# Vinmwaura/Quantized-Autoregression-Image-Generator

Hardware: NVIDIA B200
Metric: patches/sec BMU+update (SOM training step P=4 D=64 K=16384, 1 048 576 patches per step over all GPUs) (higher is better)
Workload: dtype f32 (BMU: fp16 hi/lo split x3 products on tcgen05, fp32 accumulate; update, filters and Adam fp32; filters 3xTF32)

## Files before the change

### quantized-autoregression-image-generator_b200/csrc/som_bmu_tc_l16.cu

```cuda
#include "som_common.cuh"
#include "som_tc_ptx.cuh"
#include "som_tc_split.cuh"

namespace som {
SOM_TRACE_TU(trace_set_l16)
namespace tcl16 {
using namespace tc;

constexpr int NA_MAX = 4;
constexpr int NB_MAX = 8;
constexpr int BUILD_WARP0 = 2, BUILD_WARPS = 4;
constexpr int EPI_WARP0 = 6, EPI_WARPS = 8;
constexpr int NUM_THREADS = (EPI_WARP0 + EPI_WARPS) * 32;
constexpr int A_SLOT_BYTES = 2 * A_BLK_BYTES;
constexpr int TAIL_A_BYTES = TM * 32;
constexpr int TAIL_B_BYTES = TN * 32;
constexpr int DMAX = 256;
constexpr int RING_BYTES = 192 * 1024;
constexpr int TILES_BYTES = RING_BYTES + 2 * TAIL_A_BYTES + 2 * TAIL_B_BYTES;

struct Params {
    int DB;
    int nks_last;
    int NT;
    int n_mtiles;
    int NA, NB;
    int K_pad;
    int64_t rows;
    int64_t unit_offset;
    int64_t* out_idx;
    float* out_rd;
    const void* x;
    Geom g;
    const float* scale;
    float* stage;
    const uint32_t* wflags;
};

struct __align__(8) Barriers {
    uint64_t b_full[NB_MAX], b_empty[NB_MAX];
    uint64_t t_full[2], t_empty[2];
    uint64_t a_full[NA_MAX], a_empty[NA_MAX];
    uint64_t acc_full[2], acc_empty[2];
    uint64_t exp_full[2];
    uint32_t tmem_base, pad;
};
struct Aux {
    Barriers bars;
    int foff[DMAX];
    float mrg_val[2][TM];
    int mrg_idx[2][TM];
    int row_exp[2][TM];
    alignas(8) uint8_t lo_nz[NA_MAX][8];
};
constexpr uint32_t SMEM_BYTES = 1024 + TILES_BYTES + sizeof(Aux);
constexpr int WFLAG_WORDS_MAX = 1024;
constexpr uint32_t SMEM_BYTES_W16 = SMEM_BYTES + WFLAG_WORDS_MAX * 4;
static_assert(SMEM_BYTES_W16 <= 227 * 1024, "FP16-split kernel: shared memory over the 227 KB limit");

__device__ long long g_prof16[8];

template <int CG, bool MERGED, typename T, bool W16 = false>
__global__ void __launch_bounds__(NUM_THREADS, 1)
bmu_tc_l16_kernel(const __grid_constant__ CUtensorMap map_b, const __grid_constant__ CUtensorMap map_t, const Params P) {
    constexpr bool IN16 = sizeof(T) == 2;
    pdl_launch_dependents();
    extern __shared__ uint8_t smem_raw[];
    uint8_t* tiles = aligned_tiles(smem_raw);
    constexpr int B_STAGE = B_BLK_BYTES / CG;
    constexpr int T_STAGE = TAIL_B_BYTES / CG;
    constexpr int M_STAGE = 2 * B_STAGE + T_STAGE;
    const int NA = P.NA, NB = P.NB, DB = P.DB;
    uint8_t* a_ring = tiles;
    uint8_t* a_tail = MERGED ? tiles + 2 * A_SLOT_BYTES : tiles + RING_BYTES;
    uint8_t* b_ring = MERGED ? a_tail + 2 * TAIL_A_BYTES : a_ring + (size_t)NA * A_SLOT_BYTES;
    uint8_t* t_ring = a_tail + 2 * TAIL_A_BYTES;
    Aux& aux = *reinterpret_cast<Aux*>(tiles + TILES_BYTES);
    Barriers& bars = aux.bars;
    const uint32_t rank = (CG == 2) ? cluster_ctarank() : 0u;
    const int job0 = (CG == 2) ? (int)cluster_id_x() : (int)blockIdx.x;
    const int job_stride = (CG == 2) ? (int)cluster_count_x() : (int)gridDim.x;
    const int n_jobs = (P.n_mtiles + CG - 1) / CG;

    const int warp = threadIdx.x >> 5;
    const int lane = threadIdx.x & 31;
    const int D = P.g.D;

    if (threadIdx.x == 0) {
        for (int s = 0; s < NB_MAX; ++s) { mbar_init(&bars.b_full[s], 1); mbar_init(&bars.b_empty[s], 1); }
        for (int s = 0; s < 2; ++s) { mbar_init(&bars.t_full[s], 1); mbar_init(&bars.t_empty[s], 1); }
        for (int s = 0; s < NA_MAX; ++s) { mbar_init(&bars.a_full[s], BUILD_WARPS * CG); mbar_init(&bars.a_empty[s], 1); }
        for (int a = 0; a < 2; ++a) {
            mbar_init(&bars.acc_full[a], 1);
            mbar_init(&bars.acc_empty[a], EPI_WARPS * CG);
            mbar_init(&bars.exp_full[a], BUILD_WARPS);
        }
        if (IN16)
            for (int s = 0; s < NA_MAX; ++s) *reinterpret_cast<uint64_t*>(aux.lo_nz[s]) = 0ull;
        asm volatile("fence.mbarrier_init.release.cluster;" ::: "memory");
    }
    for (int d = threadIdx.x; d < D; d += NUM_THREADS) aux.foff[d] = feat_off(P.g, d);
    if (CG == 2) {
        __syncthreads();
        cluster_sync_all();
    }
    if (warp == 1) tmem_alloc<CG>(&bars.tmem_base, 512);
    tc_fence_before();
    __syncthreads();
    if (CG == 2) cluster_sync_all();
    tc_fence_after();
    const uint32_t tmem_base = bars.tmem_base;
    pdl_wait();
    trace_stamp(s_trace_buf, 7);
    uint32_t* wbits = reinterpret_cast<uint32_t*>(tiles + TILES_BYTES + sizeof(Aux));
    if (W16) {
        for (int w = threadIdx.x; w < (P.NT * DB + 31) >> 5; w += NUM_THREADS) wbits[w] = P.wflags[w];
        __syncthreads();
    }
    auto b_lo = [&](int n, int fb) -> bool {
        if (!W16) return true;
        const int b = n * DB + fb;
        return (wbits[b >> 5] >> (b & 31)) & 1u;
    };

    if (warp == 0) {
        if (lane == 0) {
            int bs = 0, ts = 0;
            uint32_t b_ph = 0, t_ph = 0;
            const int row_off = (int)rank * (TN / CG);
            for (int q = job0; q < n_jobs; q += job_stride) {
                for (int n = 0; n < P.NT; ++n) {
                    if (MERGED) {
                        for (int fb = 0; fb < DB; ++fb) {
                            const bool blo = b_lo(n, fb);
                            mbar_wait(&bars.b_empty[bs], b_ph ^ 1);
                            if (rank == 0)
                                mbar_expect_tx(&bars.b_full[bs], (blo ? 2 : 1) * B_BLK_BYTES + (fb == 0 ? TAIL_B_BYTES : 0));
                            uint8_t* dst = b_ring + (size_t)bs * M_STAGE;
#pragma unroll
                            for (int part = 0; part < 2; ++part) {
                                if (part == 1 && !blo) break;
                                if (CG == 1) tma_load_2d(&map_b, &bars.b_full[bs], dst + part * B_STAGE, (part * DB + fb) * KBLK, n * TN);
                                else tma_load_2d_pair(&map_b, &bars.b_full[bs], dst + part * B_STAGE, (part * DB + fb) * KBLK, n * TN + row_off);
                            }
                            if (fb == 0) {
                                if (CG == 1) tma_load_2d(&map_t, &bars.b_full[bs], dst + 2 * B_STAGE, 0, n * TN);
                                else tma_load_2d_pair(&map_t, &bars.b_full[bs], dst + 2 * B_STAGE, 0, n * TN + row_off);
                            }
                            if (++bs == NB) { bs = 0; b_ph ^= 1; }
                        }
                        continue;
                    }
                    mbar_wait(&bars.t_empty[ts], t_ph ^ 1);
                    if (rank == 0) mbar_expect_tx(&bars.t_full[ts], TAIL_B_BYTES);
                    if (CG == 1) tma_load_2d(&map_t, &bars.t_full[ts], t_ring + ts * T_STAGE, 0, n * TN);
                    else tma_load_2d_pair(&map_t, &bars.t_full[ts], t_ring + ts * T_STAGE, 0, n * TN + row_off);
                    if (++ts == 2) { ts = 0; t_ph ^= 1; }
                    for (int fb = 0; fb < DB; ++fb) {
                        const bool blo = b_lo(n, fb);
#pragma unroll
                        for (int part = 0; part < 2; ++part) {
                            if (part == 1 && !blo) break;
                            mbar_wait(&bars.b_empty[bs], b_ph ^ 1);
                            if (rank == 0) mbar_expect_tx(&bars.b_full[bs], B_BLK_BYTES);
                            uint8_t* dst = b_ring + (size_t)bs * B_STAGE;
                            if (CG == 1) tma_load_2d(&map_b, &bars.b_full[bs], dst, (part * DB + fb) * KBLK, n * TN);
                            else tma_load_2d_pair(&map_b, &bars.b_full[bs], dst, (part * DB + fb) * KBLK, n * TN + row_off);
                            if (++bs == NB) { bs = 0; b_ph ^= 1; }
                        }
                    }
// ... 6 lines not shown
            if (CG == 2) mbar_wait_cluster(bar, parity); else mbar_wait(bar, parity);
        };
        const uint64_t adesc0 = umma_desc(smem_u32(a_ring));
        const uint64_t bdesc0 = umma_desc(smem_u32(b_ring));
        const uint64_t atdesc0 = umma_desc_sw32(smem_u32(a_tail));
        const uint64_t btdesc0 = umma_desc_sw32(smem_u32(t_ring));
        constexpr uint32_t A_SLOT_UNITS = (uint32_t)A_SLOT_BYTES >> 4;
        constexpr uint32_t A_LO_UNITS = (uint32_t)A_BLK_BYTES >> 4;
        constexpr uint32_t B_UNITS = (uint32_t)B_STAGE >> 4;
        constexpr uint32_t T_UNITS = (uint32_t)T_STAGE >> 4;
        constexpr uint32_t TA_UNITS = (uint32_t)TAIL_A_BYTES >> 4;
        constexpr uint32_t M_UNITS = (uint32_t)M_STAGE >> 4;
        int bs = 0, ts = 0;
        uint32_t b_ph = 0, t_ph = 0, j = 0;
        int i = 0;
        const bool prof = blockIdx.x == 0;
        long long w_acc = 0, w_b = 0, w_a = 0;
        const long long t_begin = clock64();
        auto lo_flag = [&](int as) -> uint32_t {
            return *reinterpret_cast<volatile uint64_t*>(aux.lo_nz[as]) != 0ull ? 1u : 0u;
        };
        for (int q = job0; q < n_jobs; q += job_stride, ++i) {
            uint32_t lo_mask = 0xFu;
            for (int n = 0; n < P.NT; ++n) {
                long long c0 = prof ? clock64() : 0;
                mma_wait(&bars.acc_empty[j & 1u], ((j >> 1) & 1u) ^ 1u);
                if (prof) w_acc += clock64() - c0;
                const uint32_t d_addr = tmem_base + (j & 1u) * TN;
                if (MERGED) {
                    for (int fb = 0; fb < DB; ++fb) {
                        const int nks = (fb == DB - 1) ? P.nks_last : 4;
                        const int u = i * DB + fb;
                        const int as = u % NA;
                        if (n == 0) {
                            c0 = prof ? clock64() : 0;
                            mma_wait(&bars.a_full[as], (uint32_t)(u / NA) & 1u);
                            if (prof) w_a += clock64() - c0;
                            if (IN16) lo_mask = (lo_mask & ~(1u << fb)) | (lo_flag(as) << fb);
                        }
                        const uint64_t ahi = adesc0 + (uint32_t)as * A_SLOT_UNITS;
                        const uint64_t alo = ahi + A_LO_UNITS;
                        c0 = prof ? clock64() : 0;
                        mma_wait(&bars.b_full[bs], b_ph);
                        if (prof) w_b += clock64() - c0;
                        tc_fence_after();
                        const uint64_t bhi = bdesc0 + (uint32_t)bs * M_UNITS;
                        const uint64_t blo = bhi + B_UNITS;
                        if (leader) {
                            if (fb == 0)
                                tc_mma<MmaKind::F16, CG>(d_addr, atdesc0 + (uint32_t)(i & 1) * TA_UNITS,
                                                  umma_desc_sw32(smem_u32(b_ring + (size_t)bs * M_STAGE + 2 * B_STAGE)), 0u);
#pragma unroll
                            for (int k = 0; k < 4; ++k)
                                if (k < nks) tc_mma<MmaKind::F16, CG>(d_addr, ahi + 2u * k, bhi + 2u * k, 1u);
                            if (!IN16 || ((lo_mask >> fb) & 1u)) {
#pragma unroll
                                for (int k = 0; k < 4; ++k)
                                    if (k < nks) tc_mma<MmaKind::F16, CG>(d_addr, alo + 2u * k, bhi + 2u * k, 1u);
                            }
                            if (b_lo(n, fb)) {
#pragma unroll
                                for (int k = 0; k < 4; ++k)
                                    if (k < nks) tc_mma<MmaKind::F16, CG>(d_addr, ahi + 2u * k, blo + 2u * k, 1u);
                            }
                            tc_commit<CG>(&bars.b_empty[bs]);
                            if (n == P.NT - 1) tc_commit<CG>(&bars.a_empty[as]);
                        }
                        if (++bs == NB) { bs = 0; b_ph ^= 1; }
                    }
                    if (leader) tc_commit<CG>(&bars.acc_full[j & 1u]);
                    ++j;
                    continue;
                }
                mma_wait(&bars.t_full[ts], t_ph);
                if (n == 0) {
                    const int u = i * DB;
                    mma_wait(&bars.a_full[u % NA], (uint32_t)(u / NA) & 1u);
                    if (IN16) lo_mask = (lo_mask & ~1u) | lo_flag(u % NA);
                }
                tc_fence_after();
                if (leader) {
                    tc_mma<MmaKind::F16, CG>(d_addr, atdesc0 + (uint32_t)(i & 1) * TA_UNITS, btdesc0 + (uint32_t)ts * T_UNITS, 0u);
                    tc_commit<CG>(&bars.t_empty[ts]);
                }
                if (++ts == 2) { ts = 0; t_ph ^= 1; }
                for (int fb = 0; fb < DB; ++fb) {
                    const int nks = (fb == DB - 1) ? P.nks_last : 4;
                    const int u = i * DB + fb;
                    const int as = u % NA;
// ... 18 lines not shown
                        }
                        tc_commit<CG>(&bars.b_empty[bs]);
                        if (!blo && n == P.NT - 1) tc_commit<CG>(&bars.a_empty[as]);
                    }
                    if (++bs == NB) { bs = 0; b_ph ^= 1; }
                    if (!blo) continue;
                    mma_wait(&bars.b_full[bs], b_ph);
                    tc_fence_after();
                    bd = bdesc0 + (uint32_t)bs * B_UNITS;
                    if (leader) {
#pragma unroll
                        for (int k = 0; k < 4; ++k)
                            if (k < nks) tc_mma<MmaKind::F16, CG>(d_addr, ahi + 2u * k, bd + 2u * k, 1u);
                        tc_commit<CG>(&bars.b_empty[bs]);
                        if (n == P.NT - 1) tc_commit<CG>(&bars.a_empty[as]);
                    }
                    if (++bs == NB) { bs = 0; b_ph ^= 1; }
                }
                if (leader) tc_commit<CG>(&bars.acc_full[j & 1u]);
                ++j;
            }
        }
        if (prof && leader && j > 0) {
            g_prof16[0] = clock64() - t_begin; g_prof16[1] = (long long)j;
            g_prof16[2] = w_acc; g_prof16[3] = w_b; g_prof16[4] = w_a;
        }
    } else if (warp >= BUILD_WARP0 && warp < BUILD_WARP0 + BUILD_WARPS) {
        const int t = threadIdx.x - BUILD_WARP0 * 32;
        const int vec = P.g.vec;
        const int tc_exp = (int)((__float_as_uint(__ldg(P.scale + 1)) >> 23) & 0xffu) - 127;
        const uint32_t sw = (uint32_t)(t & 7);
        float v[64];
        auto load_blk = [&](const T* src, bool ok, int fb) {
            load_row(v, src, ok, fb * 64, D, vec, [&](int d) { return aux.foff[d]; });
        };
        int i = 0;
        for (int q = job0; q < n_jobs; q += job_stride, ++i) {
            const int m = CG * q + (int)rank;
            const int64_t p = (int64_t)m * TM + t;
            const bool ok = p < P.rows;
            const T* src = static_cast<const T*>(P.x) + (ok ? patch_base(P.g, p) : 0);
            float mx = 0.f;
            for (int fb = 0; fb < DB; ++fb) {
                load_blk(src, ok, fb);
#pragma unroll
                for (int e = 0; e < 64; ++e) mx = fmaxf(mx, fabsf(v[e]));
            }
            float sp, ap;
            int es;
            f16_row_scale(mx, tc_exp, sp, ap, es);
            for (int fb = 0; fb < DB; ++fb) {
                if (DB > 1) load_blk(src, ok, fb);
                if (P.stage != nullptr && ok) {
                    float* srow = P.stage + p * D + fb * 64;
                    if ((D & 3) == 0) {
#pragma unroll
                        for (int c = 0; c < 16; ++c)
                            if (fb * 64 + c * 4 < D)
                                *reinterpret_cast<float4*>(srow + c * 4) = make_float4(v[c * 4], v[c * 4 + 1], v[c * 4 + 2], v[c * 4 + 3]);
                    } else {
#pragma unroll
                        for (int e = 0; e < 64; ++e)
                            if (fb * 64 + e < D) srow[e] = v[e];
                    }
                }
                const int u = i * DB + fb;
                const int as = u % NA;
                mbar_wait_warp<true>(&bars.a_empty[as], ((uint32_t)(u / NA) & 1u) ^ 1u, lane);
                uint8_t* hi_row = a_ring + (size_t)as * A_SLOT_BYTES + (uint32_t)t * 128u;
                uint8_t* lo_row = hi_row + A_BLK_BYTES;
                bool lo_nz = false;
#pragma unroll
                for (int c = 0; c < 8; ++c) {
                    float h[8], l[8];
#pragma unroll
                    for (int e = 0; e < 8; ++e) {
                        f16_split(v[c * 8 + e] * sp, h[e], l[e]);
                        if (IN16) lo_nz |= l[e] != 0.f;
                    }
                    const uint32_t off = (((uint32_t)c) ^ sw) << 4;
                    *reinterpret_cast<uint4*>(hi_row + off) = pack_h8(h);
                    *reinterpret_cast<uint4*>(lo_row + off) = pack_h8(l);
                }
                if (fb == 0) {
                    const uint32_t sw32 = (uint32_t)(t >> 2) & 1u;
                    uint4* rowp = reinterpret_cast<uint4*>(a_tail + (size_t)(i & 1) * TAIL_A_BYTES + t * 32);
                    const float tl[8] = {ap, ap, ap, 0.f, 0.f, 0.f, 0.f, 0.f};
                    rowp[sw32] = pack_h8(tl);
                    rowp[sw32 ^ 1u] = make_uint4(0u, 0u, 0u, 0u);
                    aux.row_exp[i & 1][t] = es;
                }
                asm volatile("fence.proxy.async.shared::cta;" ::: "memory");
                const bool warp_lo_nz = IN16 && __any_sync(0xffffffffu, lo_nz);
                __syncwarp();
                if (lane == 0) {
                    if (IN16) {
                        uint8_t* fl = &aux.lo_nz[as][rank * BUILD_WARPS + (warp - BUILD_WARP0)];
                        if (CG == 2) {
                            asm volatile(
                                "{\n"
                                ".reg .b32 ra;\n"
                                "mapa.shared::cluster.u32 ra, %0, 0;\n"
                                "st.shared::cluster.u8 [ra], %1;\n"
                                "}\n" ::"r"(smem_u32(fl)), "r"((uint32_t)warp_lo_nz)
                                : "memory");
                        } else {
                            *reinterpret_cast<volatile uint8_t*>(fl) = (uint8_t)warp_lo_nz;
                        }
                    }
                    if (CG == 2) mbar_arrive_remote(&bars.a_full[as], 0);
                    else mbar_arrive(&bars.a_full[as]);
                    if (fb == 0) mbar_arrive(&bars.exp_full[i & 1]);
                }
            }
        }
    } else if (warp >= EPI_WARP0) {
        const int half = (warp - EPI_WARP0) >> 2;
        const int lg = warp & 3;
        const int row = lg * 32 + lane;
        const int sc_exp = (int)((__float_as_uint(__ldg(P.scale)) >> 23) & 0xffu) - 127;
        uint32_t j = 0;
        int i = 0;
        for (int q = job0; q < n_jobs; q += job_stride, ++i) {
            const int m = CG * q + (int)rank;
            const int64_t p = (int64_t)m * TM + row;
            mbar_wait(&bars.exp_full[i & 1], (uint32_t)(i >> 1) & 1u);
            const int es = aux.row_exp[i & 1][row];
            float best = INFINITY;
            int bidx = 0;
            for (int n = 0; n < P.NT; ++n) {
                const uint32_t acc = j & 1u;
                mbar_wait(&bars.acc_full[acc], (j >> 1) & 1u);
                tc_fence_after();
                const uint32_t taddr = tmem_base + ((uint32_t)(lg * 32) << 16) + acc * TN + (uint32_t)half * 128u;
                const int col0 = n * TN + half * 128;
                auto consume = [&](const uint32_t (&vv)[32], int c) {
                    const float mn = min32(vv);
                    if (mn < best) { best = mn; bidx = col0 + c * 32 + first_eq32(vv, mn); }
                };
                tmem_drain<4>(taddr, consume, [&] {
                    if (lane == 0) {
                        if (CG == 2) mbar_arrive_remote_relaxed(&bars.acc_empty[acc], 0);
                        else mbar_arrive(&bars.acc_empty[acc]);
                    }
                });
                ++j;
            }
            if (half == 1) { aux.mrg_val[i & 1][row] = best; aux.mrg_idx[i & 1][row] = bidx; }
            asm volatile("bar.sync 1, 256;" ::: "memory");
            if (half == 0 && p < P.rows) {
                argmin_merge(best, bidx, aux.mrg_val[i & 1][row], aux.mrg_idx[i & 1][row]);
                P.out_idx[p] = (int64_t)bidx + P.unit_offset;
                if (P.out_rd) P.out_rd[p] = ldexpf(best, -(es + sc_exp));
            }
        }
    }

    tc_fence_before();
    __syncthreads();
    if (CG == 2) cluster_sync_all();
    if (warp == 1) {
        tc_fence_after();
        tmem_dealloc<CG>(tmem_base, 512);
    }
}

__device__ __forceinline__ void scales_from_max_norm(float mn, float* out2);
__global__ void __launch_bounds__(1024) cb_scale_l_kernel(const float* __restrict__ cn, int K, float* __restrict__ scale_out) {
    pdl_begin();
    trace_stamp(s_trace_buf, 6);
    __shared__ float sh[32];
    float mn = 0.f;
    for (int i = threadIdx.x; i < K; i += 1024) mn = fmaxf(mn, fabsf(__ldg(cn + i)));
#pragma unroll
    for (int o = 16; o > 0; o >>= 1) mn = fmaxf(mn, __shfl_xor_sync(0xffffffffu, mn, o));
    if ((threadIdx.x & 31) == 0) sh[threadIdx.x >> 5] = mn;
    __syncthreads();
    if (threadIdx.x == 0) {
        for (int w = 1; w < 32; ++w) mn = fmaxf(mn, sh[w]);
        scales_from_max_norm(mn, scale_out);
    }
}

__device__ __forceinline__ void scales_from_max_norm(float mn, float* out2) {
    const int en = (int)((__float_as_uint(mn) >> 23) & 0xffu);
    int e = 0, g = 0;
    if (mn > 0.f && en != 0xff && en != 0) {
        const int e2 = en - 127;
        const int fl = (e2 >= 0) ? (e2 >> 1) : -((1 - e2) >> 1);
        e = 7 - fl;
        e = e > 60 ? 60 : (e < -60 ? -60 : e);
        g = 14 - (e2 + e);
        g = g > 60 ? 60 : (g < -60 ? -60 : g);
    }
    out2[0] = __uint_as_float((uint32_t)(127 + e) << 23);
    out2[1] = __uint_as_float((uint32_t)(127 + g) << 23);
}

template <bool OWN_SCALE, bool W16 = false>
__global__ void __launch_bounds__(256) split_w_l16_kernel(const float* __restrict__ W, const float* __restrict__ cn,
                                                          int K, int D, int DB, int K_pad,
                                                          float* __restrict__ scale, __half* __restrict__ Bp,
                                                          __half* __restrict__ Tp, uint32_t* __restrict__ wflags) {
    pdl_begin();
    trace_stamp(s_trace_buf, 6);
    __shared__ float sh_max[8];
    __shared__ float sh_scale[2];
    if (OWN_SCALE) {
        float mn = 0.f;
        for (int i = threadIdx.x; i < K; i += 256) mn = fmaxf(mn, fabsf(__ldg(cn + i)));
#pragma unroll
        for (int o = 16; o > 0; o >>= 1) mn = fmaxf(mn, __shfl_xor_sync(0xffffffffu, mn, o));
        if ((threadIdx.x & 31) == 0) sh_max[threadIdx.x >> 5] = mn;
        __syncthreads();
        if (threadIdx.x == 0) {
            for (int w = 1; w < 8; ++w) mn = fmaxf(mn, sh_max[w]);
            scales_from_max_norm(mn, sh_scale);
            if (blockIdx.x == 0) { scale[0] = sh_scale[0]; scale[1] = sh_scale[1]; }
        }
        __syncthreads();
    }
    const int pairs = DB * 32;
    const int64_t t = blockIdx.x * (int64_t)blockDim.x + threadIdx.x;
    if (t >= (int64_t)K_pad * pairs) return;
    const int row = (int)(t / pairs);
    const int d = (int)(t - (int64_t)row * pairs) * 2;
    const int src = row < K ? row : K - 1;
    const float sc = OWN_SCALE ? sh_scale[0] : scale[0], tcs = OWN_SCALE ? sh_scale[1] : scale[1];
    float v0 = 0.f, v1 = 0.f;
    if (d < D) v0 = -2.0f * sc * W[(int64_t)src * D + d];
    if (d + 1 < D) v1 = -2.0f * sc * W[(int64_t)src * D + d + 1];
    float h0, l0, h1, l1;
    f16_split(v0, h0, l0);
    f16_split(v1, h1, l1);
    if (W16) {
        const unsigned nz = __ballot_sync(0xffffffffu, l0 != 0.f || l1 != 0.f);
        if (nz != 0u && (threadIdx.x & 31) == 0) {
            const int b = (row / TN) * DB + d / 64;
            atomicOr(wflags + (b >> 5), 1u << (b & 31));
        }
    }
    const int64_t cols = (int64_t)DB * 64;
    __half* rowp = Bp + (int64_t)row * 2 * cols;
    *reinterpret_cast<__half2*>(rowp + d) = __floats2half2_rn(h0, h1);
    *reinterpret_cast<__half2*>(rowp + cols + d) = __floats2half2_rn(l0, l1);
    if (d < 16) {
        float o0 = 0.f, o1 = 0.f;
        if (d < 4) {
            float n1, n2, n3;
            f16_norm_split3(cn[src] * sc * tcs, n1, n2, n3);
            if (d == 0) { o0 = n1; o1 = n2; } else { o0 = n3; o1 = 0.f; }
        }
        *reinterpret_cast<__half2*>(Tp + (int64_t)row * 16 + d) = __floats2half2_rn(o0, o1);
    }
}

struct Plan {
    int cg, merged, D, K, DB, nks_last, K_pad, NT, n_mtiles, NA, NB;
    size_t off_b, off_t, off_s, total;
};

static bool make_plan(Plan* pl, int64_t n, int D, int K, bool force) {
    if (D <= 16 || D > DMAX || n <= 0 || K <= 0) return false;
    pl->D = D; pl->K = K;
    pl->DB = (D + 63) / 64;
    pl->nks_last = (D - 64 * (pl->DB - 1) + 15) / 16;
    pl->K_pad = (K + TN - 1) / TN * TN;
    pl->NT = pl->K_pad / TN;
    pl->n_mtiles = (int)ceil_div64(n, TM);
    const int sms = sm_count();
    if (pl->NT < 3 || (!force && (pl->n_mtiles < sms || pl->NT < 4))) return false;
    pl->cg = (sms % 2 == 0 && pl->n_mtiles >= 2 * sms) ? 2 : 1;
    if (force && pl->DB > 2 && pl->n_mtiles >= 2 && sms % 2 == 0) pl->cg = 2;
    pl->NA = pl->DB <= 2 ? 2 : 4;
    if (pl->NA == 4 && pl->cg != 2 && !force) return false;
    pl->merged = pl->NA == 2 ? 1 : 0;
    if (pl->merged) pl->NB = (TILES_BYTES - 2 * A_SLOT_BYTES - 2 * TAIL_A_BYTES) / ((2 * B_BLK_BYTES + TAIL_B_BYTES) / pl->cg);
    else pl->NB = (RING_BYTES - pl->NA * A_SLOT_BYTES) / (B_BLK_BYTES / pl->cg);
    if (pl->NB > NB_MAX) pl->NB = NB_MAX;
    size_t o = 0;
    pl->off_b = o; o = align_up(o + (size_t)pl->K_pad * pl->DB * 64 * 2 * 2, 1024);
    pl->off_t = o; o = align_up(o + (size_t)pl->K_pad * 16 * 2, 1024);
    pl->off_s = o; o += 1024;
    pl->total = o;
    return true;
}

}

bool tc_l16_applicable(int64_t n_patches, int D, int K, bool force) {
    tcl16::Plan pl;
    return tcl16::make_plan(&pl, n_patches, D, K, force);
}

size_t tc_l16_workspace_bytes(int64_t n_patches, int D, int K, bool force) {
    tcl16::Plan pl;
    return tcl16::make_plan(&pl, n_patches, D, K, force) ? pl.total : 0;
}

bool tc_l16_plan_fields(int64_t n_patches, int D, int K, bool force, int64_t* f) {
    tcl16::Plan pl;
    if (!tcl16::make_plan(&pl, n_patches, D, K, force)) return false;
    f[PF_CG] = pl.cg;
    f[PF_MERGED] = pl.merged;
    f[PF_NT] = pl.NT;
    f[PF_DB] = pl.DB;
    f[PF_MTILES] = pl.n_mtiles;
    return true;
}

int launch_bmu_tc_l16(const void* x, int elem, const Geom& g, const float* W, const float* cn, int K,
                      int64_t unit_offset, int64_t* out_idx, float* out_rd, float* stage, void* ws, size_t ws_bytes,
                      bool force, uint32_t* wflags, cudaStream_t st) {
    using namespace tcl16;
    SOM_REQUIRE(elem == ELEM_F32 || elem == ELEM_F16 || elem == ELEM_BF16, SOM_E_BADARG, "bmu(tc f16): element type %d",
                elem);
    const int64_t n = g.n_patches;
    if (n == 0) return SOM_OK;
    Plan pl;
    SOM_REQUIRE(make_plan(&pl, n, g.D, K, force), SOM_E_UNSUPPORTED, "bmu(tc f16): shape n=%lld D=%d K=%d not covered",
                (long long)n, g.D, K);
    int rc = check_workspace(ws, ws_bytes, pl.total, "bmu(tc f16)");
    if (rc) return rc;
    __half* Bp = (__half*)((char*)ws + pl.off_b);
    __half* Tp = (__half*)((char*)ws + pl.off_t);
    float* scale = (float*)((char*)ws + pl.off_s);
    const int wwords = (pl.NT * pl.DB + 31) / 32;
    const bool w16 = wflags != nullptr && wwords <= WFLAG_WORDS_MAX;
    if (w16) {
        const cudaError_t me = cudaMemsetAsync(wflags, 0, (size_t)wwords * 4, st);
// ... 7 lines not shown
                       g.D, pl.DB, pl.K_pad, scale, Bp, Tp, wflags);
        } else {
            launch_pdl(cb_scale_l_kernel, 1, 1024, 0, st, cn, K, scale);
            rc = check_launch("cb_scale_l_kernel");
            if (rc) return rc;
            launch_pdl(w16 ? split_w_l16_kernel<false, true> : split_w_l16_kernel<false>, blocks, 256, 0, st, W, cn, K,
                       g.D, pl.DB, pl.K_pad, scale, Bp, Tp, wflags);
        }
        rc = check_launch("split_w_l16_kernel");
        if (rc) return rc;
    }
    CUtensorMap map_b, map_t;
    const uint32_t box_rows = TN / pl.cg;
    rc = make_map2d(&map_b, Bp, (uint64_t)pl.K_pad, (uint64_t)pl.DB * 64, (uint64_t)pl.DB * 64 * 4, 32, box_rows,
                    CU_TENSOR_MAP_SWIZZLE_128B);
    if (rc) return rc;
    rc = make_map2d(&map_t, Tp, (uint64_t)pl.K_pad, 8, 32, 8, box_rows, CU_TENSOR_MAP_SWIZZLE_32B);
    if (rc) return rc;

    Params P;
    P.DB = pl.DB; P.nks_last = pl.nks_last; P.NT = pl.NT; P.n_mtiles = pl.n_mtiles; P.NA = pl.NA; P.NB = pl.NB;
    P.K_pad = pl.K_pad; P.rows = n; P.unit_offset = unit_offset; P.out_idx = out_idx; P.out_rd = out_rd;
    P.x = x; P.g = g; P.scale = scale; P.stage = stage; P.wflags = wflags;

    typedef void (*KernelFn)(const CUtensorMap, const CUtensorMap, const Params);
    static const KernelFn kernels[12] = {
        bmu_tc_l16_kernel<1, false, float>, bmu_tc_l16_kernel<2, false, float>,
        bmu_tc_l16_kernel<1, true, float>, bmu_tc_l16_kernel<2, true, float>,
        bmu_tc_l16_kernel<1, false, __half>, bmu_tc_l16_kernel<2, false, __half>,
        bmu_tc_l16_kernel<1, true, __half>, bmu_tc_l16_kernel<2, true, __half>,
        bmu_tc_l16_kernel<1, false, __nv_bfloat16>, bmu_tc_l16_kernel<2, false, __nv_bfloat16>,
        bmu_tc_l16_kernel<1, true, __nv_bfloat16>, bmu_tc_l16_kernel<2, true, __nv_bfloat16>};
    static const KernelFn kernels_w16[12] = {
        bmu_tc_l16_kernel<1, false, float, true>, bmu_tc_l16_kernel<2, false, float, true>,
        bmu_tc_l16_kernel<1, true, float, true>, bmu_tc_l16_kernel<2, true, float, true>,
        bmu_tc_l16_kernel<1, false, __half, true>, bmu_tc_l16_kernel<2, false, __half, true>,
        bmu_tc_l16_kernel<1, true, __half, true>, bmu_tc_l16_kernel<2, true, __half, true>,
        bmu_tc_l16_kernel<1, false, __nv_bfloat16, true>, bmu_tc_l16_kernel<2, false, __nv_bfloat16, true>,
        bmu_tc_l16_kernel<1, true, __nv_bfloat16, true>, bmu_tc_l16_kernel<2, true, __nv_bfloat16, true>};
    static PerDeviceFlag attr_done, attr_done_w16;
    rc = w16 ? smem_opt_in(attr_done_w16, kernels_w16, 12, (int)SMEM_BYTES_W16, "bmu(tc f16)")
             : smem_opt_in(attr_done, kernels, 12, (int)SMEM_BYTES, "bmu(tc f16)");
    if (rc) return rc;
    const int n_jobs = (pl.n_mtiles + pl.cg - 1) / pl.cg;
    const int max_groups = sm_count() / pl.cg;
    const int groups = n_jobs < max_groups ? n_jobs : max_groups;
    const int ki = 4 * elem + 2 * pl.merged + pl.cg - 1;
    cudaError_t le = launch_kernel(w16 ? kernels_w16[ki] : kernels[ki], (unsigned)(groups * pl.cg), NUM_THREADS,
                                   w16 ? SMEM_BYTES_W16 : SMEM_BYTES, st, (unsigned)pl.cg, true, map_b, map_t, P);
    if (le != cudaSuccess) { set_error("bmu_tc_l16_kernel: launch: %s", cudaGetErrorString(le)); return (int)le; }
    return check_launch("bmu_tc_l16_kernel");
}

}

extern "C" SOM_API int som_debug_tc_l16_cycles(long long* out5) {
    return (int)cudaMemcpyFromSymbol(out5, som::tcl16::g_prof16, 5 * sizeof(long long));
}
```

### quantized-autoregression-image-generator_b200/csrc/som_common.cuh

```cuda
#pragma once
#include <cuda_runtime.h>
#include <stdint.h>
#include <stdio.h>
#include <stdarg.h>
#include <math.h>

#include "../../include/somcb.h"

namespace som {

void set_error(const char* fmt, ...);
int  fail(int code, const char* fmt, ...);
int  check_launch(const char* what);
unsigned long long launch_count();

#define SOM_REQUIRE(cond, code, ...) \
    do { if (!(cond)) return ::som::fail((code), __VA_ARGS__); } while (0)

int sm_count();
int current_device();

struct PerDeviceFlag {
    bool done[64] = {};
    bool pending() const { const int d = current_device(); return d < 0 || d >= 64 || !done[d]; }
// ... 8 lines not shown
    int D;
    int64_t n_patches;
    int64_t img_stride;
    int vec;
};

enum ElemType : int { ELEM_F32 = 0, ELEM_F16 = 1, ELEM_BF16 = 2 };

enum PlanFamily : int { PLAN_FFMA = 0, PLAN_S = 1, PLAN_L16 = 2, PLAN_L = 3 };
enum PlanField : int {
    PF_FAMILY,
    PF_ARITH,
    PF_CG,
    PF_MERGED,
    PF_MODE,
    PF_S,
    PF_FB_PER_SPLIT,
    PF_U,
    PF_CHUNK_ROWS,
    PF_NT,
    PF_DB,
    PF_RR,
    PF_MTILES,
    PF_COUNT
};

int make_geom(Geom* g, const void* x, int64_t n_img, int C, int H, int W, int pH, int pW, int elem_bytes = 4);

__host__ __device__ __forceinline__ int64_t patch_base(const Geom& g, int64_t p) {
    if (g.seq == 1) return p * g.img_stride;
    int64_t n = p / g.seq;
    int s = (int)(p - n * g.seq);
    int ph = s / g.gW;
    int pw = s - ph * g.gW;
    return n * g.img_stride + (int64_t)(ph * g.pH) * g.W + pw * g.pW;
}

__host__ __device__ __forceinline__ int feat_off(const Geom& g, int d) {
    if (g.seq == 1) return d;
    int pp = g.pH * g.pW;
    int c = d / pp;
    int r = d - c * pp;
    int i = r / g.pW;
    int j = r - i * g.pW;
    return (c * g.H + i) * g.W + j;
}
// ... 88 lines not shown
```

Measured before the change: 227.9 million.

## Add two-pass BMU screening: hi-only fp16 screen, candidate union, exact re-score

Replaces the single 3-product fp16-split BMU pass with a screening pipeline for the fp32 merged path. A first pass computes only the hi*hi products and keeps per-row candidate column groups within a rigorous error bound. A union kernel then builds per-job unique candidate codebook lists, and a second pass re-scores only those candidates at full 3-product precision using cp.async gathers. This aims to cut tensor-core work and B traffic for the full codebook, at the cost of two extra launches, gather loads, workspace memory and a fallback to a full scan when candidates overflow.

```diff
diff --git a/quantized-autoregression-image-generator_b200/csrc/som_bmu_tc_l16.cu b/quantized-autoregression-image-generator_b200/csrc/som_bmu_tc_l16.cu
--- a/quantized-autoregression-image-generator_b200/csrc/som_bmu_tc_l16.cu
+++ b/quantized-autoregression-image-generator_b200/csrc/som_bmu_tc_l16.cu
@@ -35,6 +35,13 @@
     const float* scale;
     float* stage;
     const uint32_t* wflags;
+    int cap;
+    int* cand;
+    int* cand_n;
+    const int* uid;
+    const int* job_nt;
+    const __half* Bp;
+    const __half* Tp;
 };
 
 struct __align__(8) Barriers {
@@ -59,8 +66,51 @@
 static_assert(SMEM_BYTES_W16 <= 227 * 1024, "FP16-split kernel: shared memory over the 227 KB limit");
 
 __device__ long long g_prof16[8];
-
-template <int CG, bool MERGED, typename T, bool W16 = false>
+__device__ long long g_prof16_scr[2][5];
+__device__ long long g_scr_stats[5];
+
+constexpr int SCR_L = 8;
+constexpr int SCR_UMAX = 4 * TN;
+constexpr int SCR_R = 8;
+constexpr int SCR_LIST_BYTES = SCR_R * 2 * TM * 12;
+__device__ __noinline__ int screen_prune(float* rv, int* rg, uint32_t* rm, int cnt, float thr) {
+    int k2 = 0;
+    for (int k = 0; k < cnt; ++k) {
+        const float v = rv[k * 2 * TM];
+        if (v <= thr) {
+            rv[k2 * 2 * TM] = v;
+            rg[k2 * 2 * TM] = rg[k * 2 * TM];
+            rm[k2 * 2 * TM] = rm[k * 2 * TM];
+            ++k2;
+        }
+    }
+    return k2;
+}
+__device__ __forceinline__ void cp_async16(uint32_t dst, const void* src) {
+    asm volatile("cp.async.cg.shared.global [%0], [%1], 16;" ::"r"(dst), "l"(src) : "memory");
+}
+
+struct ScreenAux {
+    uint64_t exp_empty[2];
+    float row_err[2][TM];
+    float best0[2][TM];
+    int cnt0[2][TM];
+};
+constexpr uint32_t SMEM_BYTES_SCR = SMEM_BYTES + sizeof(ScreenAux);
+static_assert(SMEM_BYTES_SCR <= 227 * 1024, "FP16-split screen: shared memory over the 227 KB limit");
+
+__device__ __forceinline__ float screen_err(float xx, float m2, float sc, float sp) {
+    const float X = sqrtf(xx) * (1.f + 0x1p-10f) + 0x1p-60f;
+    const float C = sc * sqrtf(m2) * (1.f + 0x1p-10f);
+    const float T = sp * sc * m2 * (1.f + 0x1p-10f);
+    const float e = (0x1p-9f + 0x1p-14f) * X * C + 0x1p-15f * (T + 3.f * X * C) + 0x1p-21f * (X + 2.f * C);
+    return e * (1.f + 0x1p-8f);
+}
+
+template <int CG>
+__device__ void screen_epilogue(const Params& P, Aux& aux, ScreenAux& sx, uint8_t* tiles, uint32_t tmem_base, int job0,
+                                int job_stride, int n_jobs, uint32_t rank, int half, int lg, int row, int lane);
+template <int CG, bool MERGED, typename T, bool W16 = false, int PASS = 0>
 __global__ void __launch_bounds__(NUM_THREADS, 1)
 bmu_tc_l16_kernel(const __grid_constant__ CUtensorMap map_b, const __grid_constant__ CUtensorMap map_t, const Params P) {
     constexpr bool IN16 = sizeof(T) == 2;
@@ -69,7 +119,9 @@
     uint8_t* tiles = aligned_tiles(smem_raw);
     constexpr int B_STAGE = B_BLK_BYTES / CG;
     constexpr int T_STAGE = TAIL_B_BYTES / CG;
-    constexpr int M_STAGE = 2 * B_STAGE + T_STAGE;
+    constexpr int T_OFF = (PASS == 1 ? 1 : 2) * B_STAGE;
+    constexpr int M_STAGE = T_OFF + T_STAGE;
+    static_assert(PASS == 0 || (MERGED && !W16 && sizeof(T) == 4), "screen: fp32 x and W, D <= 128 only");
     const int NA = P.NA, NB = P.NB, DB = P.DB;
     uint8_t* a_ring = tiles;
     uint8_t* a_tail = MERGED ? tiles + 2 * A_SLOT_BYTES : tiles + RING_BYTES;
@@ -77,6 +129,7 @@
     uint8_t* t_ring = a_tail + 2 * TAIL_A_BYTES;
     Aux& aux = *reinterpret_cast<Aux*>(tiles + TILES_BYTES);
     Barriers& bars = aux.bars;
+    ScreenAux& sx = *reinterpret_cast<ScreenAux*>(tiles + TILES_BYTES + sizeof(Aux));
     const uint32_t rank = (CG == 2) ? cluster_ctarank() : 0u;
     const int job0 = (CG == 2) ? (int)cluster_id_x() : (int)blockIdx.x;
     const int job_stride = (CG == 2) ? (int)cluster_count_x() : (int)gridDim.x;
@@ -87,7 +140,9 @@
     const int D = P.g.D;
 
     if (threadIdx.x == 0) {
-        for (int s = 0; s < NB_MAX; ++s) { mbar_init(&bars.b_full[s], 1); mbar_init(&bars.b_empty[s], 1); }
+        for (int s = 0; s < NB_MAX; ++s) { mbar_init(&bars.b_full[s], PASS == 2 ? CG : 1); mbar_init(&bars.b_empty[s], 1); }
+        if (PASS == 2)
+            for (int s = 0; s < 2; ++s) mbar_init(&sx.exp_empty[s], EPI_WARPS);
         for (int s = 0; s < 2; ++s) { mbar_init(&bars.t_full[s], 1); mbar_init(&bars.t_empty[s], 1); }
         for (int s = 0; s < NA_MAX; ++s) { mbar_init(&bars.a_full[s], BUILD_WARPS * CG); mbar_init(&bars.a_empty[s], 1); }
         for (int a = 0; a < 2; ++a) {
@@ -118,12 +173,68 @@
         __syncthreads();
     }
     auto b_lo = [&](int n, int fb) -> bool {
+        if (PASS == 1) return false;
         if (!W16) return true;
         const int b = n * DB + fb;
         return (wbits[b >> 5] >> (b & 31)) & 1u;
     };
 
-    if (warp == 0) {
+    auto job_tiles = [&](int q) -> int {
+        if (PASS != 2) return P.NT;
+        const int t = P.job_nt[q];
+        return t < 0 ? P.NT : t;
+    };
+
+    if (warp == 0 && PASS == 2) {
+        constexpr int ROWS = TN / CG;
+        int bs = 0;
+        uint32_t b_ph = 0;
+        for (int q = job0; q < n_jobs; q += job_stride) {
+            const int nt = job_tiles(q);
+            const bool full = P.job_nt[q] < 0;
+            const int* uq = P.uid + (int64_t)q * SCR_UMAX;
+            for (int n = 0; n < nt; ++n) {
+                for (int fb = 0; fb < DB; ++fb) {
+                    mbar_wait_warp<false>(&bars.b_empty[bs], b_ph ^ 1, lane);
+                    uint8_t* dst = b_ring + (size_t)bs * M_STAGE;
+                    int us[ROWS / 32];
+#pragma unroll
+                    for (int r = 0; r < ROWS / 32; ++r) {
+                        const int slot = n * TN + (int)rank * ROWS + r * 32 + lane;
+                        us[r] = full ? slot : __ldg(uq + slot);
+                    }
+#pragma unroll
+                    for (int r = 0; r < ROWS / 32; ++r) {
+                        const int t = r * 32 + lane;
+                        const int u = us[r];
+                        const uint4* src = reinterpret_cast<const uint4*>(P.Bp + (int64_t)u * DB * 128) + fb * 8;
+                        const uint32_t row = smem_u32(dst + t * 128);
+                        const uint32_t sw = (uint32_t)(t & 7);
+#pragma unroll
+                        for (int c = 0; c < 8; ++c) {
+                            cp_async16(row + ((c ^ sw) << 4), src + c);
+                            cp_async16(row + B_STAGE + ((c ^ sw) << 4), src + DB * 8 + c);
+                        }
+                        if (fb == 0) {
+                            const uint4* ts = reinterpret_cast<const uint4*>(P.Tp + (int64_t)u * 16);
+                            const uint32_t tr = smem_u32(dst + T_OFF + t * 32);
+                            const uint32_t sw32 = (uint32_t)(t >> 2) & 1u;
+                            cp_async16(tr + (sw32 << 4), ts);
+                            cp_async16(tr + ((sw32 ^ 1u) << 4), ts + 1);
+                        }
+                    }
+                    asm volatile("cp.async.wait_all;" ::: "memory");
+                    asm volatile("fence.proxy.async.shared::cta;" ::: "memory");
+                    __syncwarp();
+                    if (lane == 0) {
+                        if (CG == 2) mbar_arrive_remote(&bars.b_full[bs], 0);
+                        else mbar_arrive(&bars.b_full[bs]);
+                    }
+                    if (++bs == NB) { bs = 0; b_ph ^= 1; }
+                }
+            }
+        }
+    } else if (warp == 0) {
         if (lane == 0) {
             int bs = 0, ts = 0;
             uint32_t b_ph = 0, t_ph = 0;
@@ -144,8 +255,8 @@
                                 else tma_load_2d_pair(&map_b, &bars.b_full[bs], dst + part * B_STAGE, (part * DB + fb) * KBLK, n * TN + row_off);
                             }
                             if (fb == 0) {
-                                if (CG == 1) tma_load_2d(&map_t, &bars.b_full[bs], dst + 2 * B_STAGE, 0, n * TN);
-                                else tma_load_2d_pair(&map_t, &bars.b_full[bs], dst + 2 * B_STAGE, 0, n * TN + row_off);
+                                if (CG == 1) tma_load_2d(&map_t, &bars.b_full[bs], dst + T_OFF, 0, n * TN);
+                                else tma_load_2d_pair(&map_t, &bars.b_full[bs], dst + T_OFF, 0, n * TN + row_off);
                             }
                             if (++bs == NB) { bs = 0; b_ph ^= 1; }
                         }
@@ -198,7 +309,8 @@
         };
         for (int q = job0; q < n_jobs; q += job_stride, ++i) {
             uint32_t lo_mask = 0xFu;
-            for (int n = 0; n < P.NT; ++n) {
+            const int nt = job_tiles(q);
+            for (int n = 0; n < (PASS == 2 ? nt : P.NT); ++n) {
                 long long c0 = prof ? clock64() : 0;
                 mma_wait(&bars.acc_empty[j & 1u], ((j >> 1) & 1u) ^ 1u);
                 if (prof) w_acc += clock64() - c0;
@@ -225,11 +337,11 @@
                         if (leader) {
                             if (fb == 0)
                                 tc_mma<MmaKind::F16, CG>(d_addr, atdesc0 + (uint32_t)(i & 1) * TA_UNITS,
-                                                  umma_desc_sw32(smem_u32(b_ring + (size_t)bs * M_STAGE + 2 * B_STAGE)), 0u);
+                                                  umma_desc_sw32(smem_u32(b_ring + (size_t)bs * M_STAGE + T_OFF)), 0u);
 #pragma unroll
                             for (int k = 0; k < 4; ++k)
                                 if (k < nks) tc_mma<MmaKind::F16, CG>(d_addr, ahi + 2u * k, bhi + 2u * k, 1u);
-                            if (!IN16 || ((lo_mask >> fb) & 1u)) {
+                            if (PASS != 1 && (!IN16 || ((lo_mask >> fb) & 1u))) {
 #pragma unroll
                                 for (int k = 0; k < 4; ++k)
                                     if (k < nks) tc_mma<MmaKind::F16, CG>(d_addr, alo + 2u * k, bhi + 2u * k, 1u);
@@ -240,7 +352,7 @@
                                     if (k < nks) tc_mma<MmaKind::F16, CG>(d_addr, ahi + 2u * k, blo + 2u * k, 1u);
                             }
                             tc_commit<CG>(&bars.b_empty[bs]);
-                            if (n == P.NT - 1) tc_commit<CG>(&bars.a_empty[as]);
+                            if (n == (PASS == 2 ? nt : P.NT) - 1) tc_commit<CG>(&bars.a_empty[as]);
                         }
                         if (++bs == NB) { bs = 0; b_ph ^= 1; }
                     }
@@ -305,13 +417,15 @@
             }
         }
         if (prof && leader && j > 0) {
-            g_prof16[0] = clock64() - t_begin; g_prof16[1] = (long long)j;
-            g_prof16[2] = w_acc; g_prof16[3] = w_b; g_prof16[4] = w_a;
+            long long* g = PASS == 0 ? g_prof16 : g_prof16_scr[PASS == 0 ? 0 : PASS - 1];
+            g[0] = clock64() - t_begin; g[1] = (long long)j;
+            g[2] = w_acc; g[3] = w_b; g[4] = w_a;
         }
     } else if (warp >= BUILD_WARP0 && warp < BUILD_WARP0 + BUILD_WARPS) {
         const int t = threadIdx.x - BUILD_WARP0 * 32;
         const int vec = P.g.vec;
         const int tc_exp = (int)((__float_as_uint(__ldg(P.scale + 1)) >> 23) & 0xffu) - 127;
+        const float sc = PASS == 1 ? __ldg(P.scale) : 0.f, m2 = PASS == 1 ? __ldg(P.scale + 2) : 0.f;
         const uint32_t sw = (uint32_t)(t & 7);
         float v[64];
         auto load_blk = [&](const T* src, bool ok, int fb) {
@@ -332,6 +446,7 @@
             float sp, ap;
             int es;
             f16_row_scale(mx, tc_exp, sp, ap, es);
+            float xx = 0.f;
             for (int fb = 0; fb < DB; ++fb) {
                 if (DB > 1) load_blk(src, ok, fb);
                 if (P.stage != nullptr && ok) {
@@ -360,11 +475,15 @@
                     for (int e = 0; e < 8; ++e) {
                         f16_split(v[c * 8 + e] * sp, h[e], l[e]);
                         if (IN16) lo_nz |= l[e] != 0.f;
+                        if (PASS == 1) xx = fmaf(v[c * 8 + e] * sp, v[c * 8 + e] * sp, xx);
                     }
                     const uint32_t off = (((uint32_t)c) ^ sw) << 4;
                     *reinterpret_cast<uint4*>(hi_row + off) = pack_h8(h);
                     *reinterpret_cast<uint4*>(lo_row + off) = pack_h8(l);
                 }
+                if (PASS == 2 && fb == 0)
+                    mbar_wait_warp<true>(&sx.exp_empty[i & 1], ((uint32_t)(i >> 1) & 1u) ^ 1u, lane);
+                if (PASS == 1 && fb == DB - 1) sx.row_err[i & 1][t] = screen_err(xx, m2, sc, sp);
                 if (fb == 0) {
                     const uint32_t sw32 = (uint32_t)(t >> 2) & 1u;
                     uint4* rowp = reinterpret_cast<uint4*>(a_tail + (size_t)(i & 1) * TAIL_A_BYTES + t * 32);
@@ -393,7 +512,7 @@
                     }
                     if (CG == 2) mbar_arrive_remote(&bars.a_full[as], 0);
                     else mbar_arrive(&bars.a_full[as]);
-                    if (fb == 0) mbar_arrive(&bars.exp_full[i & 1]);
+                    if (fb == (PASS == 1 ? DB - 1 : 0)) mbar_arrive(&bars.exp_full[i & 1]);
                 }
             }
         }
@@ -404,14 +523,24 @@
         const int sc_exp = (int)((__float_as_uint(__ldg(P.scale)) >> 23) & 0xffu) - 127;
         uint32_t j = 0;
         int i = 0;
+        if (PASS == 1)
+            screen_epilogue<CG>(P, aux, sx, tiles, tmem_base, job0, job_stride, n_jobs, rank, half, lg, row, lane);
+        else
         for (int q = job0; q < n_jobs; q += job_stride, ++i) {
             const int m = CG * q + (int)rank;
             const int64_t p = (int64_t)m * TM + row;
             mbar_wait(&bars.exp_full[i & 1], (uint32_t)(i >> 1) & 1u);
             const int es = aux.row_exp[i & 1][row];
+            if (PASS == 2) {
+                __syncwarp();
+                if (lane == 0) mbar_arrive(&sx.exp_empty[i & 1]);
+            }
+            const int nt = job_tiles(q);
+            const bool full = PASS != 2 || P.job_nt[q] < 0;
+            const int* uq = PASS == 2 ? P.uid + (int64_t)q * SCR_UMAX : nullptr;
             float best = INFINITY;
             int bidx = 0;
-            for (int n = 0; n < P.NT; ++n) {
+            for (int n = 0; n < nt; ++n) {
                 const uint32_t acc = j & 1u;
                 mbar_wait(&bars.acc_full[acc], (j >> 1) & 1u);
                 tc_fence_after();
@@ -419,7 +548,12 @@
                 const int col0 = n * TN + half * 128;
                 auto consume = [&](const uint32_t (&vv)[32], int c) {
                     const float mn = min32(vv);
-                    if (mn < best) { best = mn; bidx = col0 + c * 32 + first_eq32(vv, mn); }
+                    if (PASS != 2) {
+                        if (mn < best) { best = mn; bidx = col0 + c * 32 + first_eq32(vv, mn); }
+                    } else if (mn <= best) {
+                        const int col = col0 + c * 32 + first_eq32(vv, mn);
+                        argmin_merge(best, bidx, mn, full ? col : __ldg(uq + col));
+                    }
                 };
                 tmem_drain<4>(taddr, consume, [&] {
                     if (lane == 0) {
@@ -448,6 +582,171 @@
     }
 }
 
+template <int CG>
+__device__ void screen_epilogue(const Params& P, Aux& aux, ScreenAux& sx, uint8_t* tiles, uint32_t tmem_base, int job0,
+                                int job_stride, int n_jobs, uint32_t rank, int half, int lg, int row, int lane) {
+    Barriers& bars = aux.bars;
+    const int tid = half * TM + row;
+    uint8_t* lists = tiles + TILES_BYTES - SCR_LIST_BYTES;
+    float* rv = reinterpret_cast<float*>(lists) + tid;
+    int* rg = reinterpret_cast<int*>(lists + SCR_LIST_BYTES / 3) + tid;
+    uint32_t* rm = reinterpret_cast<uint32_t*>(lists + 2 * (SCR_LIST_BYTES / 3)) + tid;
+    const int cap = P.cap;
+    uint32_t j = 0;
+    int i = 0;
+    for (int q = job0; q < n_jobs; q += job_stride, ++i) {
+        const int64_t p = (int64_t)(CG * q + (int)rank) * TM + row;
+        mbar_wait(&bars.exp_full[i & 1], (uint32_t)(i >> 1) & 1u);
+        const float e2 = 2.f * sx.row_err[i & 1][row];
+        float best = INFINITY;
+        int cnt = 0;
+        bool ovf = false;
+        for (int n = 0; n < P.NT; ++n) {
+            const uint32_t acc = j & 1u;
+            mbar_wait(&bars.acc_full[acc], (j >> 1) & 1u);
+            tc_fence_after();
+            const uint32_t taddr = tmem_base + ((uint32_t)(lg * 32) << 16) + acc * TN + (uint32_t)half * 128u;
+            const int col0 = n * TN + half * 128;
+            auto consume = [&](const uint32_t (&vv)[32], int c) {
+                const float mn = min32(vv);
+                best = fminf(best, mn);
+                const float thr = best + e2;
+                if (mn <= thr) {
+                    uint32_t m = 0;
+#pragma unroll
+                    for (int e = 0; e < 32; ++e) m |= (__uint_as_float(vv[e]) <= thr ? 1u : 0u) << e;
+                    if (cnt < SCR_R) {
+                        rv[cnt * 2 * TM] = mn;
+                        rg[cnt * 2 * TM] = (col0 >> 5) + c;
+                        rm[cnt * 2 * TM] = m;
+                        ++cnt;
+                    } else {
+                        ovf = true;
+                    }
+                }
+            };
+            tmem_drain<4>(taddr, consume, [&] {
+                if (lane == 0) {
+                    if (CG == 2) mbar_arrive_remote_relaxed(&bars.acc_empty[acc], 0);
+                    else mbar_arrive(&bars.acc_empty[acc]);
+                }
+            });
+            ++j;
+            if (cnt > SCR_R - 4) cnt = screen_prune(rv, rg, rm, cnt, best + e2);
+        }
+        if (half == 0) sx.best0[i & 1][row] = best;
+        else aux.mrg_val[i & 1][row] = best;
+        asm volatile("bar.sync 1, 256;" ::: "memory");
+        const float rbest = fminf(sx.best0[i & 1][row], aux.mrg_val[i & 1][row]);
+        const float thr = rbest + e2;
+        ovf = ovf || !(fabsf(rbest) <= 3.4e38f && e2 <= 3.4e38f);
+        int units = 0;
+        if (!ovf) {
+            cnt = screen_prune(rv, rg, rm, cnt, thr);
+            for (int k = 0; k < cnt; ++k) units += __popc(rm[k * 2 * TM]);
+        }
+        if (half == 0) sx.cnt0[i & 1][row] = ovf ? cap + 1 : units;
+        asm volatile("bar.sync 1, 256;" ::: "memory");
+        if (p < P.rows) {
+            const int c0 = half == 0 ? 0 : sx.cnt0[i & 1][row];
+            const bool over = ovf || c0 + units > cap;
+            if (!over) {
+                int* out = P.cand + p * SCR_L + c0;
+                for (int k = 0; k < cnt; ++k)
+                    for (uint32_t m = rm[k * 2 * TM]; m != 0u; m &= m - 1u) *out++ = rg[k * 2 * TM] * 32 + __ffs(m) - 1;
+            }
+            if (half == 1) P.cand_n[p] = over ? cap + 1 : c0 + units;
+        }
+    }
+}
+
+__global__ void __launch_bounds__(256) screen_union_kernel(const int* __restrict__ cand, const int* __restrict__ cand_n,
+                                                           int64_t rows, int rows_per_job, int cap,
+                                                           int* __restrict__ uid, int* __restrict__ job_nt,
+                                                           long long* __restrict__ stats) {
+    pdl_begin();
+    constexpr int NK = 2 * TM * SCR_L;
+    __shared__ int key[NK];
+    __shared__ int wsum[8];
+    const int q = blockIdx.x, t = threadIdx.x;
+    const int64_t p = (int64_t)q * rows_per_job + t;
+    int c = 0;
+    bool ov = false;
+    if (t < rows_per_job && p < rows) {
+        c = cand_n[p];
+        ov = c > cap;
+    }
+#pragma unroll
+    for (int k = 0; k < SCR_L; ++k) key[k * 256 + t] = (!ov && k < c) ? cand[p * SCR_L + k] : INT_MAX;
+    if (__syncthreads_or(ov)) {
+        if (t == 0) {
+            job_nt[q] = -1;
+            if (stats) { atomicAdd((unsigned long long*)stats + 2, 1ull); atomicAdd((unsigned long long*)stats + 4, 1ull); }
+        }
+        return;
+    }
+    if (stats) {
+        const int rv = __syncthreads_count(t < rows_per_job && p < rows);
+        const int cs = __syncthreads_count(c & 1) + 2 * __syncthreads_count(c & 2) + 4 * __syncthreads_count(c & 4) +
+                       8 * __syncthreads_count(c & 8);
+        if (t == 0) {
+            atomicAdd((unsigned long long*)stats, (unsigned long long)rv);
+            atomicAdd((unsigned long long*)stats + 1, (unsigned long long)cs);
+        }
+    }
+    const int n = __syncthreads_or(c > 4) ? NK : __syncthreads_or(c > 2) ? NK / 2 : __syncthreads_or(c > 1) ? NK / 4 : NK / 8;
+    for (int size = 2; size <= n; size <<= 1) {
+        for (int stride = size >> 1; stride > 0; stride >>= 1) {
+            __syncthreads();
+            for (int h = t; h < n / 2; h += 256) {
+                const int lo = 2 * stride * (h / stride) + (h % stride), hi = lo + stride;
+                const int a = key[lo], b = key[hi];
+                if ((a > b) == ((lo & size) == 0)) { key[lo] = b; key[hi] = a; }
+            }
+        }
+    }
+    __syncthreads();
+    int keep = 0, last = -1;
+#pragma unroll
+    for (int e = 0; e < 8; ++e) {
+        const int h = 8 * t + e, k = key[h];
+        if (k != INT_MAX && (h == 0 || key[h - 1] != k)) { ++keep; last = k; }
+    }
+    int incl = keep;
+#pragma unroll
+    for (int o = 1; o < 32; o <<= 1) {
+        const int v = __shfl_up_sync(0xffffffffu, incl, o);
+        if ((t & 31) >= o) incl += v;
+    }
+    if ((t & 31) == 31) wsum[t >> 5] = incl;
+    __syncthreads();
+    int base = 0, total = 0;
+    for (int w = 0; w < 8; ++w) { if (w < (t >> 5)) base += wsum[w]; total += wsum[w]; }
+    int off = base + incl - keep;
+    int* uq = uid + (int64_t)q * SCR_UMAX;
+    if (total > SCR_UMAX || total == 0) {
+        if (t == 0) {
+            job_nt[q] = -1;
+            if (stats) { atomicAdd((unsigned long long*)stats + 2, 1ull); atomicAdd((unsigned long long*)stats + 4, 1ull); }
+        }
+        return;
+    }
+#pragma unroll
+    for (int e = 0; e < 8; ++e) {
+        const int h = 8 * t + e, k = key[h];
+        if (k != INT_MAX && (h == 0 || key[h - 1] != k)) uq[off++] = k;
+    }
+    const int nt = (total + TN - 1) / TN;
+    __syncthreads();
+    if (keep > 0 && off == total) wsum[0] = last;
+    __syncthreads();
+    for (int h = total + t; h < nt * TN; h += 256) uq[h] = wsum[0];
+    if (t == 0) {
+        job_nt[q] = nt;
+        if (stats) { atomicAdd((unsigned long long*)stats + 2, 1ull); atomicAdd((unsigned long long*)stats + 3, (unsigned long long)total); }
+    }
+}
+
 __device__ __forceinline__ void scales_from_max_norm(float mn, float* out2);
 __global__ void __launch_bounds__(1024) cb_scale_l_kernel(const float* __restrict__ cn, int K, float* __restrict__ scale_out) {
     pdl_begin();
@@ -462,6 +761,7 @@
     if (threadIdx.x == 0) {
         for (int w = 1; w < 32; ++w) mn = fmaxf(mn, sh[w]);
         scales_from_max_norm(mn, scale_out);
+        scale_out[2] = mn;
     }
 }
 
@@ -499,7 +799,7 @@
         if (threadIdx.x == 0) {
             for (int w = 1; w < 8; ++w) mn = fmaxf(mn, sh_max[w]);
             scales_from_max_norm(mn, sh_scale);
-            if (blockIdx.x == 0) { scale[0] = sh_scale[0]; scale[1] = sh_scale[1]; }
+            if (blockIdx.x == 0) { scale[0] = sh_scale[0]; scale[1] = sh_scale[1]; scale[2] = mn; }
         }
         __syncthreads();
     }
@@ -540,8 +840,13 @@
 
 struct Plan {
     int cg, merged, D, K, DB, nks_last, K_pad, NT, n_mtiles, NA, NB;
+    int NB1;
     size_t off_b, off_t, off_s, total;
+    size_t off_cand, off_cn, off_uid, off_jn;
 };
+
+static int s_screen_mode = 1;
+static bool s_screen_stats = false;
 
 static bool make_plan(Plan* pl, int64_t n, int D, int K, bool force) {
     if (D <= 16 || D > DMAX || n <= 0 || K <= 0) return false;
@@ -561,10 +866,19 @@
     if (pl->merged) pl->NB = (TILES_BYTES - 2 * A_SLOT_BYTES - 2 * TAIL_A_BYTES) / ((2 * B_BLK_BYTES + TAIL_B_BYTES) / pl->cg);
     else pl->NB = (RING_BYTES - pl->NA * A_SLOT_BYTES) / (B_BLK_BYTES / pl->cg);
     if (pl->NB > NB_MAX) pl->NB = NB_MAX;
+    pl->NB1 = (TILES_BYTES - 2 * A_SLOT_BYTES - 2 * TAIL_A_BYTES - SCR_LIST_BYTES) / ((B_BLK_BYTES + TAIL_B_BYTES) / pl->cg);
+    if (pl->NB1 > NB_MAX) pl->NB1 = NB_MAX;
     size_t o = 0;
     pl->off_b = o; o = align_up(o + (size_t)pl->K_pad * pl->DB * 64 * 2 * 2, 1024);
     pl->off_t = o; o = align_up(o + (size_t)pl->K_pad * 16 * 2, 1024);
     pl->off_s = o; o += 1024;
+    if (pl->merged) {
+        const int64_t jobs = ((int64_t)pl->n_mtiles + pl->cg - 1) / pl->cg;
+        pl->off_cand = o; o = align_up(o + (size_t)n * SCR_L * 4, 1024);
+        pl->off_cn = o; o = align_up(o + (size_t)n * 4, 1024);
+        pl->off_uid = o; o = align_up(o + (size_t)jobs * SCR_UMAX * 4, 1024);
+        pl->off_jn = o; o = align_up(o + (size_t)jobs * 4, 1024);
+    }
     pl->total = o;
     return true;
 }
@@ -589,6 +903,7 @@
     f[PF_NT] = pl.NT;
     f[PF_DB] = pl.DB;
     f[PF_MTILES] = pl.n_mtiles;
+    f[PF_SCREEN] = pl.merged && tcl16::s_screen_mode != 0;
     return true;
 }
 
@@ -642,6 +957,7 @@
     P.DB = pl.DB; P.nks_last = pl.nks_last; P.NT = pl.NT; P.n_mtiles = pl.n_mtiles; P.NA = pl.NA; P.NB = pl.NB;
     P.K_pad = pl.K_pad; P.rows = n; P.unit_offset = unit_offset; P.out_idx = out_idx; P.out_rd = out_rd;
     P.x = x; P.g = g; P.scale = scale; P.stage = stage; P.wflags = wflags;
+    P.cap = 0; P.cand = nullptr; P.cand_n = nullptr; P.uid = nullptr; P.job_nt = nullptr; P.Bp = nullptr; P.Tp = nullptr;
 
     typedef void (*KernelFn)(const CUtensorMap, const CUtensorMap, const Params);
     static const KernelFn kernels[12] = {
@@ -658,13 +974,47 @@
         bmu_tc_l16_kernel<1, true, __half, true>, bmu_tc_l16_kernel<2, true, __half, true>,
         bmu_tc_l16_kernel<1, false, __nv_bfloat16, true>, bmu_tc_l16_kernel<2, false, __nv_bfloat16, true>,
         bmu_tc_l16_kernel<1, true, __nv_bfloat16, true>, bmu_tc_l16_kernel<2, true, __nv_bfloat16, true>};
+    const int n_jobs = (pl.n_mtiles + pl.cg - 1) / pl.cg;
+    const int max_groups = sm_count() / pl.cg;
+    const int groups = n_jobs < max_groups ? n_jobs : max_groups;
+    if (elem == ELEM_F32 && !w16 && pl.merged && s_screen_mode != 0) {
+        static const KernelFn kernels_scr[4] = {
+            bmu_tc_l16_kernel<1, true, float, false, 1>, bmu_tc_l16_kernel<2, true, float, false, 1>,
+            bmu_tc_l16_kernel<1, true, float, false, 2>, bmu_tc_l16_kernel<2, true, float, false, 2>};
+        static PerDeviceFlag attr_done_scr;
+        rc = smem_opt_in(attr_done_scr, kernels_scr, 4, (int)SMEM_BYTES_SCR, "bmu(tc f16 screen)");
+        if (rc) return rc;
+        char* w = (char*)ws;
+        P.cap = s_screen_mode == 2 ? 0 : SCR_L;
+        P.cand = (int*)(w + pl.off_cand);
+        P.cand_n = (int*)(w + pl.off_cn);
+        P.uid = (const int*)(w + pl.off_uid);
+        P.job_nt = (const int*)(w + pl.off_jn);
+        P.Bp = Bp;
+        P.Tp = Tp;
+        P.NB = pl.NB1;
+        cudaError_t le = launch_kernel(kernels_scr[pl.cg - 1], (unsigned)(groups * pl.cg), NUM_THREADS, SMEM_BYTES_SCR, st,
+                                       (unsigned)pl.cg, true, map_b, map_t, P);
+        if (le != cudaSuccess) { set_error("bmu_tc_l16_kernel (screen): launch: %s", cudaGetErrorString(le)); return (int)le; }
+        rc = check_launch("bmu_tc_l16_kernel (screen)");
+        if (rc) return rc;
+        long long* stats = nullptr;
+        if (s_screen_stats) cudaGetSymbolAddress((void**)&stats, g_scr_stats);
+        launch_pdl(screen_union_kernel, (unsigned)n_jobs, 256, 0, st, (const int*)P.cand, (const int*)P.cand_n, n,
+                   pl.cg * TM, P.cap, (int*)P.uid, (int*)P.job_nt, stats);
+        rc = check_launch("screen_union_kernel");
+        if (rc) return rc;
+        P.NB = pl.NB;
+        P.stage = nullptr;
+        le = launch_kernel(kernels_scr[2 + pl.cg - 1], (unsigned)(groups * pl.cg), NUM_THREADS, SMEM_BYTES_SCR, st,
+                           (unsigned)pl.cg, true, map_b, map_t, P);
+        if (le != cudaSuccess) { set_error("bmu_tc_l16_kernel (re-score): launch: %s", cudaGetErrorString(le)); return (int)le; }
+        return check_launch("bmu_tc_l16_kernel (re-score)");
+    }
     static PerDeviceFlag attr_done, attr_done_w16;
     rc = w16 ? smem_opt_in(attr_done_w16, kernels_w16, 12, (int)SMEM_BYTES_W16, "bmu(tc f16)")
              : smem_opt_in(attr_done, kernels, 12, (int)SMEM_BYTES, "bmu(tc f16)");
     if (rc) return rc;
-    const int n_jobs = (pl.n_mtiles + pl.cg - 1) / pl.cg;
-    const int max_groups = sm_count() / pl.cg;
-    const int groups = n_jobs < max_groups ? n_jobs : max_groups;
     const int ki = 4 * elem + 2 * pl.merged + pl.cg - 1;
     cudaError_t le = launch_kernel(w16 ? kernels_w16[ki] : kernels[ki], (unsigned)(groups * pl.cg), NUM_THREADS,
                                    w16 ? SMEM_BYTES_W16 : SMEM_BYTES, st, (unsigned)pl.cg, true, map_b, map_t, P);
@@ -677,3 +1027,20 @@
 extern "C" SOM_API int som_debug_tc_l16_cycles(long long* out5) {
     return (int)cudaMemcpyFromSymbol(out5, som::tcl16::g_prof16, 5 * sizeof(long long));
 }
+
+extern "C" SOM_API int som_debug_l16_screen(int mode) {
+    const int prev = som::tcl16::s_screen_mode;
+    if (mode >= 0 && mode <= 2) som::tcl16::s_screen_mode = mode;
+    return prev;
+}
+
+extern "C" SOM_API int som_debug_l16_screen_stats(long long* out15, int reset) {
+    if (reset) {
+        som::tcl16::s_screen_stats = true;
+        const long long z[5] = {0, 0, 0, 0, 0};
+        return (int)cudaMemcpyToSymbol(som::tcl16::g_scr_stats, z, sizeof(z));
+    }
+    cudaError_t e = cudaMemcpyFromSymbol(out15, som::tcl16::g_prof16_scr, 10 * sizeof(long long));
+    if (e == cudaSuccess) e = cudaMemcpyFromSymbol(out15 + 10, som::tcl16::g_scr_stats, 5 * sizeof(long long));
+    return (int)e;
+}
diff --git a/quantized-autoregression-image-generator_b200/csrc/som_common.cuh b/quantized-autoregression-image-generator_b200/csrc/som_common.cuh
--- a/quantized-autoregression-image-generator_b200/csrc/som_common.cuh
+++ b/quantized-autoregression-image-generator_b200/csrc/som_common.cuh
@@ -54,6 +54,7 @@
     PF_DB,
     PF_RR,
     PF_MTILES,
+    PF_SCREEN,
     PF_COUNT
 };
 
```

New measurement: 247.2 million (median of 6 runs). 8.4% higher.
